# mlaprise/mfrec

Hardware: NVIDIA B200
Metric: rating_updates_per_s (higher is better)
Workload: dtype f32

## Files before the change

### mfrec_b200/csrc/sgd.cu

```cuda
#include <algorithm>
#include <cmath>
#include <cstdlib>
#include <cstring>
#include <thread>
#include <type_traits>

#include <cuda_bf16.h>
#include <cuda_fp16.h>

#include "common.cuh"

namespace {

constexpr int kChunk = 64;
constexpr int kStages = 4;
constexpr int kDepth = 16;
constexpr int kQuadsAhead = kDepth / 4;
constexpr int kRing = kChunk * kStages;
static_assert(kChunk % 4 == 0, "chunks must be 16-byte multiples");
static_assert(4 * kDepth <= kChunk, "the prefetch cursor may run at most one chunk ahead");

struct SgdRank {
    const PackedRating *packed;
    const int64_t *bucket_off;
    const int32_t *col_start;
    float *Q, *ib, *P, *ub;
    double *se_part;
    int32_t *ticks;
    float *peer_Q, *peer_ib;
    int32_t *peer_ticks;
    int32_t *abort;
    int rank;
};

struct SgdParams {
    SgdRank self;
    const SgdRank *ranks;
    int64_t it_begin, it_end;
    int64_t e_base;
    int se_stride;
    int B, W, G, world;
    int tile_rows;
    float lr, Ku, Ki, Kb;
    int update_users, update_items;
    float fx_scale, fx_inv;
    unsigned long long wait_ns;
};

template <int BYTES>
__device__ __forceinline__ void cp_async(void *dst_smem, const void *src_gmem)
{
    if constexpr (BYTES == 16)
        asm volatile("cp.async.cg.shared.global [%0], [%1], 16;" ::"r"(smem_u32(dst_smem)), "l"(src_gmem) : "memory");
    else
        asm volatile("cp.async.ca.shared.global [%0], [%1], %2;" ::"r"(smem_u32(dst_smem)), "l"(src_gmem), "n"(BYTES) : "memory");
}
__device__ __forceinline__ void cp_async_commit() { asm volatile("cp.async.commit_group;" ::: "memory"); }
template <int N>
__device__ __forceinline__ void cp_async_wait() { asm volatile("cp.async.wait_group %0;" ::"n"(N) : "memory"); }

template <int E>
struct Frag {
    static constexpr int V = E >= 4 ? 4 : E;
    static constexpr int NV = E / V;
    float x[E];
};

template <int E>
__device__ __forceinline__ void frag_load(Frag<E> &f, const float *row, int lane)
{
    constexpr int V = Frag<E>::V, NV = Frag<E>::NV;
#pragma unroll
    for (int c = 0; c < NV; ++c) {
        const float *p = row + (c * 32 + lane) * V;
        if constexpr (V == 4) {
            const float4 t = *reinterpret_cast<const float4 *>(p);
            f.x[c * 4 + 0] = t.x; f.x[c * 4 + 1] = t.y; f.x[c * 4 + 2] = t.z; f.x[c * 4 + 3] = t.w;
        } else if constexpr (V == 2) {
            const float2 t = *reinterpret_cast<const float2 *>(p);
            f.x[0] = t.x; f.x[1] = t.y;
        } else {
            f.x[0] = *p;
        }
    }
}

template <int E>
__device__ __forceinline__ void frag_store(const Frag<E> &f, float *row, int lane)
{
    constexpr int V = Frag<E>::V, NV = Frag<E>::NV;
#pragma unroll
    for (int c = 0; c < NV; ++c) {
        float *p = row + (c * 32 + lane) * V;
        if constexpr (V == 4)
            *reinterpret_cast<float4 *>(p) = make_float4(f.x[c * 4], f.x[c * 4 + 1], f.x[c * 4 + 2], f.x[c * 4 + 3]);
        else if constexpr (V == 2)
            *reinterpret_cast<float2 *>(p) = make_float2(f.x[0], f.x[1]);
        else
            *p = f.x[0];
    }
}

template <int E>
__device__ __forceinline__ void frag_store_lane(const Frag<E> &f, float *p)
{
    constexpr int V = Frag<E>::V, NV = Frag<E>::NV;
#pragma unroll
    for (int c = 0; c < NV; ++c) {
        if constexpr (V == 4)
            *reinterpret_cast<float4 *>(p + c * 128) = make_float4(f.x[c * 4], f.x[c * 4 + 1], f.x[c * 4 + 2], f.x[c * 4 + 3]);
        else if constexpr (V == 2)
            *reinterpret_cast<float2 *>(p) = make_float2(f.x[0], f.x[1]);
        else
            *p = f.x[0];
    }
}

template <typename T>
__device__ __forceinline__ T *row_ptr(T *base, uint32_t idx, uint32_t stride_bytes)
{
    uint64_t a;
    asm("mad.wide.u32 %0, %1, %2, %3;" : "=l"(a) : "r"(idx), "r"(stride_bytes), "l"(base));
    return reinterpret_cast<T *>(a);
}

template <int E, typename PT>
__device__ __forceinline__ void pfrag_load(Frag<E> &f, const PT *row, int lane)
{
    if constexpr (sizeof(PT) == 4) {
        frag_load<E>(f, reinterpret_cast<const float *>(row), lane);
    } else {
        constexpr int V = Frag<E>::V, NV = Frag<E>::NV;
        static_assert(V >= 2, "16-bit rows need at least two elements per lane");
#pragma unroll
        for (int c = 0; c < NV; ++c) {
            const PT *p = row + (c * 32 + lane) * V;
#pragma unroll
            for (int h = 0; h < V / 2; ++h) {
                float2 t;
                if constexpr (std::is_same<PT, __half>::value)
                    t = __half22float2(*reinterpret_cast<const __half2 *>(p + 2 * h));
                else
                    t = __bfloat1622float2(*reinterpret_cast<const __nv_bfloat162 *>(p + 2 * h));
                f.x[c * V + 2 * h] = t.x;
                f.x[c * V + 2 * h + 1] = t.y;
            }
        }
    }
}

template <int E, typename PT>
__device__ __forceinline__ void pfrag_store_lane(const Frag<E> &f, PT *p, uint32_t &rng)
{
    if constexpr (sizeof(PT) == 4) {
        frag_store_lane<E>(f, reinterpret_cast<float *>(p));
    } else {
        constexpr int V = Frag<E>::V, NV = Frag<E>::NV;
#pragma unroll
        for (int c = 0; c < NV; ++c) {
            uint32_t w[V / 2];
#pragma unroll
            for (int h = 0; h < V / 2; ++h) {
                const float a = f.x[c * V + 2 * h], b = f.x[c * V + 2 * h + 1];
                if constexpr (std::is_same<PT, __half>::value) {
                    const __half2 t = __floats2half2_rn(a, b);
                    w[h] = *reinterpret_cast<const uint32_t *>(&t);
                } else {
                    rng = rng * 1664525u + 1013904223u;
                    const uint32_t ua = __float_as_uint(a) + (rng & 0xffffu);
                    const uint32_t ub = __float_as_uint(b) + (rng >> 16);
                    w[h] = (ua >> 16) | (ub & 0xffff0000u);
                }
            }
            PT *q = p + c * 32 * V;
            if constexpr (V == 4) *reinterpret_cast<uint2 *>(q) = make_uint2(w[0], w[1]);
            else *reinterpret_cast<uint32_t *>(q) = w[0];
        }
    }
}

__device__ __forceinline__ unsigned long long pack2(float lo, float hi)
{
    unsigned long long r;
    asm("mov.b64 %0, {%1, %2};" : "=l"(r) : "f"(lo), "f"(hi));
    return r;
}
__device__ __forceinline__ void unpack2(unsigned long long v, float &lo, float &hi)
{
    asm("mov.b64 {%0, %1}, %2;" : "=f"(lo), "=f"(hi) : "l"(v));
}
__device__ __forceinline__ unsigned long long mul2(unsigned long long a, unsigned long long b)
{
    unsigned long long r;
    asm("mul.rn.f32x2 %0, %1, %2;" : "=l"(r) : "l"(a), "l"(b));
    return r;
}
__device__ __forceinline__ unsigned long long fma2(unsigned long long a, unsigned long long b, unsigned long long c)
{
    unsigned long long r;
    asm("fma.rn.f32x2 %0, %1, %2, %3;" : "=l"(r) : "l"(a), "l"(b), "l"(c));
    return r;
}

__device__ __forceinline__ int ld_acquire_sys(const int32_t *p)
{
    int v;
    asm volatile("ld.acquire.sys.global.s32 %0, [%1];" : "=r"(v) : "l"(p) : "memory");
    return v;
}
__device__ __forceinline__ void st_release_sys(int32_t *p, int v)
{
    asm volatile("st.release.sys.global.s32 [%0], %1;" ::"l"(p), "r"(v) : "memory");
}
__device__ __forceinline__ unsigned long long global_ns()
{
    unsigned long long t;
    asm volatile("mov.u64 %0, %globaltimer;" : "=l"(t));
    return t;
}

template <int E, int KERNEL, int MAXT, bool GATED, bool RING, typename PT = float>
__global__ void __launch_bounds__(MAXT, 1)
sgd_block_kernel(const SgdParams prm)
{
    constexpr int KPAD = E * 32;
    constexpr unsigned FULL = 0xffffffffu;
    extern __shared__ __align__(128) unsigned char smem_raw[];
    const int W = prm.W;
    const int warp = threadIdx.x >> 5, lane = threadIdx.x & 31;
    const int rb = RING ? (int)(blockIdx.x % (unsigned)prm.B) : (int)blockIdx.x;
    const SgdRank R = RING ? prm.ranks[blockIdx.x / (unsigned)prm.B] : prm.self;
    __shared__ int abort_s;

    float *Qs = reinterpret_cast<float *>(smem_raw);
    float *ibs = Qs + (size_t)prm.tile_rows * KPAD;
    PT *prow_all = reinterpret_cast<PT *>(ibs + ((prm.tile_rows + 3) & ~3));
    float *pbias_all = reinterpret_cast<float *>(prow_all + (size_t)W * kDepth * KPAD);
    PackedRating *ring_all = reinterpret_cast<PackedRating *>(pbias_all + (size_t)W * kDepth);
    uint64_t *bars = reinterpret_cast<uint64_t *>(ring_all + (size_t)W * kRing);
    int64_t *boff = reinterpret_cast<int64_t *>(bars + 1 + kStages * W);
    double *se_s = reinterpret_cast<double *>(boff + W * W + 2);
    volatile int32_t *phase_done = reinterpret_cast<volatile int32_t *>(se_s + W);

    PT *prow = prow_all + (size_t)warp * kDepth * KPAD;
    float *pbias = pbias_all + warp * kDepth;
    PackedRating *ring = ring_all + (size_t)warp * kRing;
    uint64_t *tile_bar = bars;
    uint64_t *my_bar = bars + 1 + kStages * warp;

    if (threadIdx.x == 0) {
        mbar_init(tile_bar, 1);
        for (int i = 0; i < kStages * W; ++i) mbar_init(bars + 1 + i, 1);
        for (int i = 0; i < W; ++i) phase_done[i] = 0;
        abort_s = 0;
        asm volatile("fence.mbarrier_init.release.cluster;" ::: "memory");
    }

    const float lr = prm.lr;
    const bool upd_u = !GATED || prm.update_users != 0, upd_i = !GATED || prm.update_items != 0;
    const float a_i = upd_i ? 1.f - prm.lr * prm.Ki : 1.f;
    const float a_u = upd_u ? 1.f - prm.lr * prm.Ku : 1.f;
    const float a_b = 1.f - prm.lr * prm.Kb;
    const unsigned long long a_i2 = pack2(a_i, a_i), a_u2 = pack2(a_u, a_u);
    const bool upd_bu = (KERNEL == MFREC_KERNEL_LINEAR) || upd_u;
    const bool upd_bi = (KERNEL == MFREC_KERNEL_LINEAR) || upd_i;
    const float fx_scale = prm.fx_scale, fx_inv = prm.fx_inv;
    constexpr uint32_t kRowBytes = KPAD * sizeof(PT);
    PT *const P_rows = reinterpret_cast<PT *>(R.P);
    PT *const P_lane = P_rows + lane * Frag<E>::V;
    uint32_t rng = 0x9e3779b9u * (blockIdx.x * 1024u + threadIdx.x + 1u);
    float *const ub_g = R.ub;
    const int64_t steps_per_epoch = (int64_t)prm.G * prm.B;

    double se = 0.0;
    uint32_t chunk_seq = 0;
    uint32_t tile_seq = 0;
    bool chunks_issued = false;

    int s, t_slab, epoch_rel;
    {
        const int64_t e0 = prm.it_begin / steps_per_epoch;
        const int in0 = (int)(prm.it_begin - e0 * steps_per_epoch);
        epoch_rel = (int)(e0 - prm.e_base);
        t_slab = in0 / prm.B;
        s = in0 - t_slab * prm.B;
    }
    for (int64_t it = prm.it_begin; it < prm.it_end; ++it) {
        const int step = (int)(it - prm.it_begin);
        const int in_epoch = t_slab * prm.B + s;
        int slab = R.rank + t_slab;
        if (slab >= prm.G) slab -= prm.G;
        int cbl = rb + s;
        if (cbl >= prm.B) cbl -= prm.B;
        const int cbg = slab * prm.B + cbl;
        const int cs = R.col_start[cbg * W];
        const int nq = R.col_start[(cbg + 1) * W] - cs;
        const int tick_need = RING ? (int)it : epoch_rel * prm.B + s;

        const int64_t bucket_base = (((int64_t)slab * prm.B + rb) * prm.B + cbl) * W * W;
        for (int i = threadIdx.x; i <= W * W; i += blockDim.x) boff[i] = R.bucket_off[bucket_base + i];
        if (threadIdx.x == 0) {
            if (R.ticks) {
                if constexpr (RING) {
                    const unsigned long long t0 = global_ns();
                    uint32_t polls = 0;
                    while (ld_acquire_sys(R.ticks + cbg) < tick_need) {
                        __nanosleep(128);
                        if ((++polls & 1023u) == 0) {
                            if (*(volatile int32_t *)R.abort) { abort_s = 1; break; }
                            if (prm.wait_ns && global_ns() - t0 > prm.wait_ns) {
                                *(volatile int32_t *)R.abort = 1;
                                abort_s = 1;
                                break;
                            }
                        }
                    }
                } else {
                    while (ld_acquire_gpu(R.ticks + cbg) < tick_need) __nanosleep(64);
                }
                asm volatile("fence.proxy.async;" ::: "memory");
            }
            bool go = nq > 0;
            if constexpr (RING) go = go && !abort_s;
            if (go) {
                const uint32_t total = (uint32_t)nq * KPAD * 4u;
                mbar_expect_tx(tile_bar, total);
                const char *src = reinterpret_cast<const char *>(R.Q + (size_t)cs * KPAD);
                char *dst = reinterpret_cast<char *>(Qs);
                for (uint32_t o = 0; o < total; o += 32768u)
                    bulk_g2s(dst + o, src + o, min(32768u, total - o), tile_bar);
            }
        }
        __syncthreads();
        if constexpr (RING) {
            if (abort_s) break;
        }

        const int64_t S0 = boff[warp * W];
        const uint32_t slen = (uint32_t)(boff[warp * W + W] - S0);
        const uint32_t nchunks = (slen + kChunk - 1) / kChunk;
        const uint32_t nquads = slen / 4;
        const PackedRating *stream = R.packed + S0;
        const int64_t *off_w = boff + warp * W;

        constexpr uint32_t kRingQ = kRing / 4, kChunkQ = kChunk / 4;
        static_assert((kRingQ & (kRingQ - 1)) == 0 && (kChunkQ & (kChunkQ - 1)) == 0 &&
                      (kQuadsAhead & (kQuadsAhead - 1)) == 0, "ring sizes must be powers of two");
        const uint32_t base_q = (chunk_seq % kStages) * kChunkQ;
        const char *const ring_b = reinterpret_cast<const char *>(ring);
        auto quad_rec = [&](uint32_t x) { return ring_b + ((base_q + x) & (kRingQ - 1)) * 48u; };
        auto chunk_wait = [&](uint32_t c) {
            const uint32_t g = chunk_seq + c;
            mbar_wait(my_bar + (g % kStages), (g / kStages) & 1u);
        };
        auto issue_chunk = [&](uint32_t c) {
            if (lane == 0) {
                const uint32_t cnt = min((uint32_t)kChunk, slen - c * kChunk);
                const uint32_t g = chunk_seq + c;
                uint64_t *bar = my_bar + (g % kStages);
                mbar_expect_tx(bar, cnt * 12u);
                bulk_g2s(ring + (g % kStages) * kChunk, stream + (size_t)c * kChunk, cnt * 12u, bar);
            }
        };
        if (!chunks_issued)
            for (uint32_t c = 0; c < nchunks && c < (uint32_t)kStages; ++c) issue_chunk(c);

        PT *const prow_lane = prow + lane * Frag<E>::V;
        for (uint32_t fx = 0; fx + 1 < (uint32_t)kQuadsAhead; ++fx) {
            if (fx < nquads) {
                if ((fx & (kChunkQ - 1)) == 0) chunk_wait(fx / kChunkQ);
                const char *rec = quad_rec(fx);
                const uint32_t fslot0 = (fx & (kQuadsAhead - 1)) * 4;
#pragma unroll
                for (int t = 0; t < 4; ++t) {
                    const uint32_t ut = *reinterpret_cast<const uint32_t *>(rec + 12 * t) & kIdMask;
                    const PT *gsrc = row_ptr(P_lane, ut, kRowBytes);
#pragma unroll
                    for (int c = 0; c < Frag<E>::NV; ++c)
                        cp_async<Frag<E>::V * sizeof(PT)>(prow_lane + (fslot0 + t) * KPAD + c * 32 * Frag<E>::V,
                                                          gsrc + c * 32 * Frag<E>::V);
                }
                if (lane < 4) {
                    const uint32_t ul = *reinterpret_cast<const uint32_t *>(rec + 12 * lane) & kIdMask;
                    cp_async<4>(pbias + fslot0 + lane, row_ptr(ub_g, ul, 4));
                }
            }
            cp_async_commit();
        }

        if (nq > 0) {
            mbar_wait(tile_bar, tile_seq & 1u);
            tile_seq += 1;
        }
        for (int i = threadIdx.x; i < nq; i += blockDim.x) ibs[i] = __ldcg(R.ib + cs + i);
        __syncthreads();

        Frag<E> cp, cq;
#pragma unroll
        for (int e = 0; e < E; ++e) { cp.x[e] = 0.f; cq.x[e] = 0.f; }
        float cbu = 0.f, cbi = 0.f, se_f = 0.f;
        int prev_u = -1, prev_i = -1;

        auto warp_sum_fx = [&](int v) { return __reduce_add_sync(FULL, v); };
        auto dot_fx = [&](const Frag<E> &pu, const Frag<E> &q) {
            float part;
            if constexpr (E >= 2) {
                unsigned long long acc = mul2(pack2(pu.x[0], pu.x[1]), pack2(q.x[0], q.x[1]));
#pragma unroll
                for (int e = 2; e < E; e += 2)
                    acc = fma2(pack2(pu.x[e], pu.x[e + 1]), pack2(q.x[e], q.x[e + 1]), acc);
                float lo, hi;
                unpack2(acc, lo, hi);
                part = lo + hi;
            } else {
                part = pu.x[0] * q.x[0];
            }
            return __float2int_rn(part * fx_scale);
        };
        auto apply = [&](int isum, float r, Frag<E> &pu, float &bu, Frag<E> &q, float &bi) {
            const float pred = fmaf((float)isum, fx_inv, bi + bu);
            float err, grad;
            if constexpr (KERNEL == MFREC_KERNEL_LINEAR) {
                err = r - pred;
                grad = err;
            } else {
                const float sig = 1.f / (1.f + expf(-pred));
                err = r - (1.f + 4.f * sig);
                grad = err * sig * (1.f - sig) * 4.f;
            }
            se_f = fmaf(err, err, se_f);
            const float gl = lr * grad;
            bu = upd_bu ? fmaf(a_b, bu, gl) : bu;
            bi = upd_bi ? fmaf(a_b, bi, gl) : bi;
            const float gli = upd_i ? gl : 0.f, glu = upd_u ? gl : 0.f;
            if constexpr (E >= 2) {
                const unsigned long long glu2 = pack2(glu, glu), gli2 = pack2(gli, gli);
#pragma unroll
                for (int e = 0; e < E; e += 2) {
                    const unsigned long long pe = pack2(pu.x[e], pu.x[e + 1]), qe = pack2(q.x[e], q.x[e + 1]);
                    unpack2(fma2(glu2, qe, mul2(a_u2, pe)), pu.x[e], pu.x[e + 1]);
                    unpack2(fma2(gli2, pe, mul2(a_i2, qe)), q.x[e], q.x[e + 1]);
                }
            } else {
                const float pe = pu.x[0], qe = q.x[0];
                pu.x[0] = fmaf(glu, qe, a_u * pe);
                q.x[0] = fmaf(gli, pe, a_i * qe);
            }
        };
        auto store_p_row = [&](int u, const Frag<E> &pu) {
            pfrag_store_lane<E, PT>(pu, row_ptr(P_lane, (uint32_t)u, kRowBytes), rng);
        };
        auto store_p = [&](int u, const Frag<E> &pu, float bu) {
            store_p_row(u, pu);
            if (lane == 0) *row_ptr(ub_g, (uint32_t)u, 4) = bu;
        };
        auto store_bias_quad = [&](const int (&u4)[4], const float (&b4)[4], uint32_t keep) {
            const bool lo = (lane & 2) == 0, even = (lane & 1) == 0;
            const int ul = lo ? (even ? u4[0] : u4[1]) : (even ? u4[2] : u4[3]);
            const float v = lo ? (even ? b4[0] : b4[1]) : (even ? b4[2] : b4[3]);
            if (lane < 4 && ((keep >> lane) & 1u)) *row_ptr(ub_g, (uint32_t)ul, 4) = v;
        };
        auto store_q = [&](int it, const Frag<E> &q, float bi) {
            frag_store<E>(q, Qs + (size_t)(it - cs) * KPAD, lane);
            if (lane == 0) ibs[it - cs] = bi;
        };

        auto update_one = [&](uint32_t slot, int u, int it, float r, bool stale) {
            Frag<E> pu;
            float bu;
            if (u == prev_u) {
#pragma unroll
                for (int e = 0; e < E; ++e) pu.x[e] = cp.x[e];
                bu = cbu;
            } else if (stale) {
                __syncwarp();
                pfrag_load<E, PT>(pu, row_ptr(P_rows, (uint32_t)u, kRowBytes), lane);
                bu = *row_ptr(ub_g, (uint32_t)u, 4);
            } else {
                pfrag_load<E, PT>(pu, prow + slot * KPAD, lane);
                bu = pbias[slot];
            }
            if (it != prev_i) {
                frag_load<E>(cq, Qs + (size_t)(it - cs) * KPAD, lane);
                cbi = ibs[it - cs];
            }
            const int isum = warp_sum_fx(dot_fx(pu, cq));
            apply(isum, r, pu, bu, cq, cbi);
            store_q(it, cq, cbi);
            store_p(u, pu, bu);
#pragma unroll
            for (int e = 0; e < E; ++e) cp.x[e] = pu.x[e];
            cbu = bu;
            prev_u = u;
            prev_i = it;
        };

        auto load_quad_p = [&](uint32_t slot0, Frag<E> (&p4)[4], float (&b4)[4]) {
#pragma unroll
            for (int t = 0; t < 4; ++t) {
                pfrag_load<E, PT>(p4[t], prow + (slot0 + t) * KPAD, lane);
                b4[t] = pbias[slot0 + t];
            }
        };
        auto chain_quad = [&](uint32_t slot0, const int (&u4)[4], int it, const float (&r4)[4], auto &&hook) {
            Frag<E> p4[4];
            float b4[4];
            load_quad_p(slot0, p4, b4);
            if (it != prev_i) {
                frag_load<E>(cq, Qs + (size_t)(it - cs) * KPAD, lane);
                cbi = ibs[it - cs];
            }
#pragma unroll
            for (int t = 0; t < 4; ++t) {
                const int isum = warp_sum_fx(dot_fx(p4[t], cq));
                hook(t);
                apply(isum, r4[t], p4[t], b4[t], cq, cbi);
                store_p_row(u4[t], p4[t]);
            }
            store_bias_quad(u4, b4, 0xfu);
            store_q(it, cq, cbi);
#pragma unroll
            for (int e = 0; e < E; ++e) cp.x[e] = p4[3].x[e];
            cbu = b4[3];
            prev_u = u4[3];
            prev_i = it;
        };
        auto indep_quad = [&](uint32_t slot0, const int (&u4)[4], const int (&i4)[4], const float (&r4)[4], auto &&hook) {
            Frag<E> p4[4], q4[4];
            float b4[4], c4[4];
            load_quad_p(slot0, p4, b4);
#pragma unroll
            for (int t = 0; t < 4; ++t) {
                frag_load<E>(q4[t], Qs + (size_t)(i4[t] - cs) * KPAD, lane);
                c4[t] = ibs[i4[t] - cs];
            }
            int f[4], sm[4];
#pragma unroll
            for (int t = 0; t < 4; ++t) f[t] = dot_fx(p4[t], q4[t]);
#pragma unroll
            for (int t = 0; t < 4; ++t) sm[t] = warp_sum_fx(f[t]);
#pragma unroll
            for (int t = 0; t < 4; ++t) hook(t);
#pragma unroll
            for (int t = 0; t < 4; ++t) apply(sm[t], r4[t], p4[t], b4[t], q4[t], c4[t]);
#pragma unroll
            for (int t = 0; t < 4; ++t) {
                store_q(i4[t], q4[t], c4[t]);
                store_p_row(u4[t], p4[t]);
            }
            store_bias_quad(u4, b4, 0xfu);
#pragma unroll
            for (int e = 0; e < E; ++e) { cp.x[e] = p4[3].x[e]; cq.x[e] = q4[3].x[e]; }
            cbu = b4[3];
            cbi = c4[3];
            prev_u = u4[3];
            prev_i = i4[3];
        };
        auto clean_quad = [&](uint32_t slot0, const int (&u4)[4], const int (&i4)[4], const int (&f4)[4],
                              const float (&r4)[4], auto &&hook) {
            Frag<E> p4[4];
            float b4[4];
            load_quad_p(slot0, p4, b4);
#pragma unroll
            for (int t = 0; t < 4; ++t) {
                if (f4[t] & kFlagAdjUser) {
#pragma unroll
                    for (int e = 0; e < E; ++e) p4[t].x[e] = t ? p4[t ? t - 1 : 0].x[e] : cp.x[e];
                    b4[t] = t ? b4[t ? t - 1 : 0] : cbu;
                }
                if (i4[t] != prev_i) {
                    frag_load<E>(cq, Qs + (size_t)(i4[t] - cs) * KPAD, lane);
                    cbi = ibs[i4[t] - cs];
                }
                prev_i = i4[t];
                const int isum = warp_sum_fx(dot_fx(p4[t], cq));
                hook(t);
                apply(isum, r4[t], p4[t], b4[t], cq, cbi);
                store_q(i4[t], cq, cbi);
                store_p_row(u4[t], p4[t]);
            }
            {
                uint32_t keep = 0x8u;
#pragma unroll
                for (int t = 0; t < 3; ++t) keep |= (f4[t + 1] & kFlagAdjUser) ? 0u : (1u << t);
                store_bias_quad(u4, b4, keep);
            }
#pragma unroll
            for (int e = 0; e < E; ++e) cp.x[e] = p4[3].x[e];
            cbu = b4[3];
            prev_u = u4[3];
            prev_i = i4[3];
        };

        const int32_t done_base = step * W;
        uint32_t x = 0;
        int4 na = make_int4(0, 0, 0, 0), nb = na, nc = na;
        if (nquads > 0) {
            const int4 *nsrc = reinterpret_cast<const int4 *>(quad_rec(0));
            na = nsrc[0]; nb = nsrc[1]; nc = nsrc[2];
        }
        for (int p = 0; p < W; ++p) {
            const uint32_t xe = (uint32_t)(off_w[p + 1] - S0) >> 2;
            if (p > 0) {
                const volatile int32_t *flag = phase_done + (warp + 1 == W ? 0 : warp + 1);
                if (lane == 0) {
                    while (*flag < done_base + p) __nanosleep(32);
                    __threadfence_block();
                }
                __syncwarp();
            }
            se_f = 0.f;
#pragma unroll 1
            for (; x < xe; ++x) {
                if ((x & (kChunkQ - 1)) == 0 && x != 0) {
                    const uint32_t nc = x / kChunkQ - 1 + kStages;
                    if (nc < nchunks) {
                        __syncwarp();
                        issue_chunk(nc);
                    }
                }
                const uint32_t fx = x + (kQuadsAhead - 1);
                if ((fx & (kChunkQ - 1)) == 0 && fx < nquads) chunk_wait(fx / kChunkQ);
                const char *const frec = quad_rec(min(fx, nquads - 1));
                const uint32_t fu[4] = {*reinterpret_cast<const uint32_t *>(frec) & kIdMask,
                                        *reinterpret_cast<const uint32_t *>(frec + 12) & kIdMask,
                                        *reinterpret_cast<const uint32_t *>(frec + 24) & kIdMask,
                                        *reinterpret_cast<const uint32_t *>(frec + 36) & kIdMask};
                const uint32_t fslot0 = (fx & (kQuadsAhead - 1)) * 4;
                PT *const fdst = prow_lane + fslot0 * KPAD;
                auto fetch_row = [&](int t) {
                    const PT *gsrc = row_ptr(P_lane, fu[t], kRowBytes);
#pragma unroll
                    for (int c = 0; c < Frag<E>::NV; ++c)
                        cp_async<Frag<E>::V * sizeof(PT)>(fdst + t * KPAD + c * 32 * Frag<E>::V, gsrc + c * 32 * Frag<E>::V);
                };
                cp_async_wait<kQuadsAhead - 2>();
                __syncwarp();
                const int4 a = na, b = nb, c2 = nc;
                {
                    const int4 *nsrc = reinterpret_cast<const int4 *>(quad_rec(x + 1));
                    na = nsrc[0]; nb = nsrc[1]; nc = nsrc[2];
                }
                const uint32_t slot0 = (x & (kQuadsAhead - 1)) * 4;
                const int u4[4] = {a.x & kIdMask, a.w & kIdMask, b.z & kIdMask, c2.y & kIdMask};
                const int f4[4] = {a.y, b.x, b.w, c2.z};
                const int i4[4] = {a.y & kIdMask, b.x & kIdMask, b.w & kIdMask, c2.z & kIdMask};
                const float r4[4] = {__int_as_float(a.z), __int_as_float(b.y), __int_as_float(c2.x), __int_as_float(c2.w)};
                const int qtype = (a.x >> kQuadShift) & 3;
                if (qtype == kQuadIndep) {
                    indep_quad(slot0, u4, i4, r4, fetch_row);
                } else if (qtype == kQuadChain) {
                    chain_quad(slot0, u4, i4[0], r4, fetch_row);
                } else if (qtype == kQuadClean) {
                    clean_quad(slot0, u4, i4, f4, r4, fetch_row);
                } else {
#pragma unroll
                    for (int t = 0; t < 4; ++t) {
                        if (!(f4[t] & kFlagPad)) update_one(slot0 + t, u4[t], i4[t], r4[t], (f4[t] & kFlagStale) != 0);
                        fetch_row(t);
                    }
                }
                {
                    const bool lo = (lane & 2) == 0, even = (lane & 1) == 0;
                    const uint32_t ul = lo ? (even ? fu[0] : fu[1]) : (even ? fu[2] : fu[3]);
                    if (lane < 4) cp_async<4>(pbias + fslot0 + lane, row_ptr(ub_g, ul, 4));
                }
                cp_async_commit();
            }
            se += (double)se_f;
            prev_i = -1;
            __syncwarp();
            if (lane == 0) {
                __threadfence_block();
                phase_done[warp] = done_base + p + 1;
            }
        }
        cp_async_wait<0>();
        chunk_seq += nchunks;
        chunks_issued = false;
        int ns = s + 1, nt = t_slab;
        if (ns == prm.B) {
            ns = 0;
            nt = t_slab + 1 == prm.G ? 0 : t_slab + 1;
        }
        if (it + 1 < prm.it_end) {
            int nslab = R.rank + nt;
            if (nslab >= prm.G) nslab -= prm.G;
            int ncbl = rb + ns;
            if (ncbl >= prm.B) ncbl -= prm.B;
            const int64_t nbase = ((((int64_t)nslab * prm.B + rb) * prm.B + ncbl) * W + warp) * W;
            const int64_t nS0 = __ldg(R.bucket_off + nbase);
            const uint32_t nslen = (uint32_t)(__ldg(R.bucket_off + nbase + W) - nS0);
            const uint32_t nn = min((nslen + kChunk - 1) / kChunk, (uint32_t)kStages);
            if (lane == 0) {
                for (uint32_t c = 0; c < nn; ++c) {
                    const uint32_t cnt = min((uint32_t)kChunk, nslen - c * kChunk);
                    const uint32_t g = chunk_seq + c;
                    uint64_t *bar = my_bar + (g % kStages);
                    mbar_expect_tx(bar, cnt * 12u);
                    bulk_g2s(ring + (g % kStages) * kChunk, R.packed + nS0 + (size_t)c * kChunk, cnt * 12u, bar);
                }
            }
            chunks_issued = true;
        }
        __syncthreads();
        const bool to_peer = RING && s + 1 == prm.B && prm.world > 1;
        {
            const int nvec = nq * KPAD / 4;
            float4 *dst = reinterpret_cast<float4 *>((to_peer ? R.peer_Q : R.Q) + (size_t)cs * KPAD);
            float *dst_b = (to_peer ? R.peer_ib : R.ib) + cs;
            const float4 *srcv = reinterpret_cast<const float4 *>(Qs);
            float chk = 0.f;
            for (int i = threadIdx.x; i < nvec; i += blockDim.x) {
                const float4 t = srcv[i];
                chk = fmaf(0.f, t.x, fmaf(0.f, t.y, fmaf(0.f, t.z, fmaf(0.f, t.w, chk))));
                dst[i] = t;
            }
            for (int i = threadIdx.x; i < nq; i += blockDim.x) {
                chk = fmaf(0.f, ibs[i], chk);
                dst_b[i] = ibs[i];
            }
            if (__any_sync(FULL, chk != chk)) se = NAN;
        }
        const bool epoch_ends = in_epoch + 1 == (int)steps_per_epoch || it + 1 == prm.it_end;
        if (epoch_ends) {
            if (lane == 0) se_s[warp] = se;
            se = 0.0;
        }
        if (R.ticks) {
            if constexpr (RING) {
                if (to_peer) {
                    __threadfence_system();
                    __syncthreads();
                    if (threadIdx.x == 0) st_release_sys(R.peer_ticks + cbg, tick_need + 1);
                } else {
                    __threadfence();
                    __syncthreads();
                    if (threadIdx.x == 0) st_release_gpu(R.ticks + cbg, tick_need + 1);
                }
            } else {
                __threadfence();
                __syncthreads();
                if (threadIdx.x == 0) st_release_gpu(R.ticks + cbg, tick_need + 1);
            }
        } else {
            __syncthreads();
        }
        if (epoch_ends && threadIdx.x == 0) {
            double tot = 0.0;
            for (int w = 0; w < W; ++w) tot += se_s[w];
            R.se_part[(int64_t)epoch_rel * prm.se_stride + rb] = tot;
        }
        if (ns == 0 && nt == 0) epoch_rel += 1;
        s = ns;
        t_slab = nt;
    }
    if constexpr (RING) {
        if (abort_s && threadIdx.x == 0) {
            const int64_t e_last = (prm.it_end - 1) / steps_per_epoch;
            for (int64_t e = prm.e_base; e <= e_last; ++e) R.se_part[(e - prm.e_base) * prm.se_stride + rb] = NAN;
        }
    }
}

__global__ void __launch_bounds__(1024) se_reduce_kernel(const double *__restrict__ part, int64_t n,
                                                         double *__restrict__ out)
{
    __shared__ double sh[1024];
    double acc = 0.0;
    for (int64_t i = threadIdx.x; i < n; i += 1024) acc += part[i];
    sh[threadIdx.x] = acc;
    __syncthreads();
    for (int o = 512; o > 0; o >>= 1) {
        if ((int)threadIdx.x < o) sh[threadIdx.x] += sh[threadIdx.x + o];
        __syncthreads();
    }
    if (threadIdx.x == 0) *out = sh[0];
}

__global__ void __launch_bounds__(256)
merge_copies_kernel(float *__restrict__ Q, float *__restrict__ ib, int kpad, const int32_t *__restrict__ hot_off,
                    const int32_t *__restrict__ hot_rows, int32_t n_hot, int32_t row_lo, int32_t row_hi,
                    const int32_t *ticks, int32_t tick_lo, int32_t tick_hi, int32_t tick_need,
                    int32_t *abort_flag, unsigned long long wait_ns)
{
    __shared__ int ok;
    if (ticks) {
        if (threadIdx.x == 0) {
            ok = 1;
            const unsigned long long t0 = global_ns();
            for (int32_t c = tick_lo; c < tick_hi && ok; ++c) {
                uint32_t polls = 0;
                while (ld_acquire_sys(ticks + c) < tick_need) {
                    __nanosleep(256);
                    if ((++polls & 255u) == 0 &&
                        (*(volatile int32_t *)abort_flag || (wait_ns && global_ns() - t0 > wait_ns))) {
                        *(volatile int32_t *)abort_flag = 1;
                        ok = 0;
                        break;
                    }
                }
            }
        }
        __syncthreads();
        if (!ok) return;
    }
    const int lane = threadIdx.x & 31;
    const int64_t warps = ((int64_t)gridDim.x * blockDim.x) >> 5;
    for (int64_t h = ((int64_t)blockIdx.x * blockDim.x + threadIdx.x) >> 5; h < n_hot; h += warps) {
        const int32_t a = hot_off[h], b = hot_off[h + 1];
        const int32_t first = hot_rows[a];
        if (first < row_lo || first >= row_hi) continue;
        const float inv = 1.f / (float)(b - a);
        for (int c = lane; c < kpad; c += 32) {
            float acc = 0.f;
            for (int32_t j = a; j < b; ++j) acc += __ldcg(Q + (size_t)hot_rows[j] * kpad + c);
            acc *= inv;
            for (int32_t j = a; j < b; ++j) Q[(size_t)hot_rows[j] * kpad + c] = acc;
        }
        if (lane == 0) {
            float acc = 0.f;
            for (int32_t j = a; j < b; ++j) acc += __ldcg(ib + hot_rows[j]);
            acc *= inv;
            for (int32_t j = a; j < b; ++j) ib[hot_rows[j]] = acc;
        }
    }
}

constexpr int kSeqRegs = 32;

__global__ void __launch_bounds__(32)
kmf_sequential_kernel(int kernel, int nbr_epochs, int dim, double lr, double K_users,
                      double K_items, double K_bias, double *u, double *v,
                      const int32_t *idx, const double *ratings, int64_t nnz,
                      int64_t ni, int64_t nu, double *ib, double *ub,
                      int update_users, int update_items, double *rmse_out)
{
    if (blockIdx.x != 0) return;
    const int lane = threadIdx.x;
    const unsigned FULLM = 0xffffffffu;
    for (int epoch = 0; epoch < nbr_epochs; ++epoch) {
        double se = 0.0;
        int2 ui = make_int2(0, 0);
        double rating = 0.0;
        if (lane < nnz) { ui = reinterpret_cast<const int2 *>(idx)[lane]; rating = ratings[lane]; }
        for (int64_t base = 0; base < nnz; base += 32) {
            const int cnt = (int)(nnz - base < 32 ? nnz - base : 32);
            const bool live = lane < cnt;
            const int user = ui.x, item = ui.y;
            const double r = rating;
            {
                const int64_t j = base + 32 + lane;
                if (j < nnz) { ui = reinterpret_cast<const int2 *>(idx)[j]; rating = ratings[j]; }
            }
            int lmax;
            const int level = mfrec_window_levels(user, item, live, lane, lmax);
            double e2 = 0.0;
            for (int L = 1; L <= lmax; ++L) {
                if (live && level == L) {
                    double *const ui_ = u + item, *const vu_ = v + user;
                    const double bi0 = ib[item], bu0 = ub[user];
                    double s = __dadd_rn(__dadd_rn(0.0, bi0), bu0);
                    auto err_grad = [&](double &err, double &grad) {
                        if (kernel == MFREC_KERNEL_LINEAR) {
                            err = __dadd_rn(r, -s);
                            grad = err;
                        } else {
                            const double sig = 1.0 / __dadd_rn(1.0, exp(-s));
                            const double p = __dadd_rn(1.0, __dmul_rn(sig, 4.0));
                            err = __dadd_rn(r, -p);
                            grad = __dmul_rn(__dmul_rn(__dmul_rn(err, sig), __dadd_rn(1.0, -sig)), 4.0);
                        }
                        e2 = __dmul_rn(err, err);
                        if (kernel == MFREC_KERNEL_LINEAR || update_users)
                            ub[user] = __dadd_rn(bu0, __dmul_rn(lr, __dadd_rn(grad, -__dmul_rn(K_bias, bu0))));
                        if (kernel == MFREC_KERNEL_LINEAR || update_items)
                            ib[item] = __dadd_rn(bi0, __dmul_rn(lr, __dadd_rn(grad, -__dmul_rn(K_bias, bi0))));
                    };
                    double err, grad;
                    if (dim <= kSeqRegs) {
                        double mf[kSeqRegs], cf[kSeqRegs];
#pragma unroll
                        for (int f = 0; f < kSeqRegs; ++f)
                            if (f < dim) { mf[f] = ui_[(int64_t)f * ni]; cf[f] = vu_[(int64_t)f * nu]; }
#pragma unroll
                        for (int f = 0; f < kSeqRegs; ++f)
                            if (f < dim) s = __dadd_rn(s, __dmul_rn(mf[f], cf[f]));
                        err_grad(err, grad);
#pragma unroll
                        for (int f = 0; f < kSeqRegs; ++f) {
                            if (f >= dim) continue;
                            if (update_items)
                                ui_[(int64_t)f * ni] =
                                    __dadd_rn(mf[f], __dmul_rn(lr, __dadd_rn(__dmul_rn(grad, cf[f]), -__dmul_rn(K_items, mf[f]))));
                            if (update_users)
                                vu_[(int64_t)f * nu] =
                                    __dadd_rn(cf[f], __dmul_rn(lr, __dadd_rn(__dmul_rn(grad, mf[f]), -__dmul_rn(K_users, cf[f]))));
                        }
                    } else {
                        for (int f0 = 0; f0 < dim; f0 += 8) {
                            double a[8], b[8];
#pragma unroll
                            for (int j = 0; j < 8; ++j)
                                if (f0 + j < dim) { a[j] = ui_[(int64_t)(f0 + j) * ni]; b[j] = vu_[(int64_t)(f0 + j) * nu]; }
#pragma unroll
                            for (int j = 0; j < 8; ++j)
                                if (f0 + j < dim) s = __dadd_rn(s, __dmul_rn(a[j], b[j]));
                        }
                        err_grad(err, grad);
                        for (int f0 = 0; f0 < dim; f0 += 8) {
                            double mf[8], cf[8];
#pragma unroll
                            for (int j = 0; j < 8; ++j)
                                if (f0 + j < dim) { mf[j] = ui_[(int64_t)(f0 + j) * ni]; cf[j] = vu_[(int64_t)(f0 + j) * nu]; }
#pragma unroll
                            for (int j = 0; j < 8; ++j) {
                                if (f0 + j >= dim) continue;
                                if (update_items)
                                    ui_[(int64_t)(f0 + j) * ni] =
                                        __dadd_rn(mf[j], __dmul_rn(lr, __dadd_rn(__dmul_rn(grad, cf[j]), -__dmul_rn(K_items, mf[j]))));
                                if (update_users)
                                    vu_[(int64_t)(f0 + j) * nu] =
                                        __dadd_rn(cf[j], __dmul_rn(lr, __dadd_rn(__dmul_rn(grad, mf[j]), -__dmul_rn(K_users, cf[j]))));
                            }
                        }
                    }
                }
                __syncwarp();
            }
            for (int t = 0; t < cnt; ++t) se = __dadd_rn(se, __shfl_sync(FULLM, e2, t));
        }
        if (rmse_out && lane == 0) rmse_out[epoch] = sqrt(se / (double)nnz);
        __syncwarp();
    }
}

}

size_t mfrec_sgd_smem_bytes(int tile_rows, int kpad, int W, int p_elem_bytes)
{
    size_t b = (size_t)tile_rows * kpad * 4;
    b += (size_t)((tile_rows + 3) & ~3) * 4;
    b += (size_t)W * kDepth * kpad * p_elem_bytes;
    b += (size_t)W * kDepth * 4;
    b += (size_t)W * kRing * sizeof(PackedRating);
    b += (size_t)(1 + kStages * W) * 8;
    b += (size_t)(W * W + 2) * 8;
    b += (size_t)W * 8;
    b += (size_t)((W + 3) & ~3) * 4;
    return b + 384;
}

namespace {

template <int E>
int launch_sgd(mfrec_ctx *ctx, int kernel, SgdParams &prm, size_t smem, bool cooperative, int grid, bool ring,
               int p_kind)
{
    const bool wide = prm.W > 8;
    const bool gated = !(prm.update_users && prm.update_items);
    void (*fn)(const SgdParams) = nullptr;
    const bool mid = prm.W > 8 && prm.W <= 12 && !gated;
#define MF_PICK(K)                                                                                     \
    fn = mid ? sgd_block_kernel<E, K, 384, false, false>                                                \
       : wide ? (gated ? sgd_block_kernel<E, K, 512, true, false> : sgd_block_kernel<E, K, 512, false, false>) \
              : (gated ? sgd_block_kernel<E, K, 256, true, false> : sgd_block_kernel<E, K, 256, false, false>)
#define MF_PICK_RING(K) \
    fn = mid ? sgd_block_kernel<E, K, 384, false, true>                                                  \
       : wide ? sgd_block_kernel<E, K, 512, false, true> : sgd_block_kernel<E, K, 256, false, true>
    if (p_kind != MFREC_STORAGE_F32) {
        if constexpr (E >= 2) {
            if (ring || gated || prm.W > 12)
                return mfrec_set_error(ctx, MFREC_ERR_UNSUPPORTED,
                                       "fp16 / bf16 user-factor storage: single device, both sides updated, at most 12 warps per CTA");
#define MF_PICK16(K, T) fn = prm.W > 8 ? sgd_block_kernel<E, K, 384, false, false, T> : sgd_block_kernel<E, K, 256, false, false, T>
            if (kernel == MFREC_KERNEL_LINEAR) {
                if (p_kind == MFREC_STORAGE_F16) { MF_PICK16(MFREC_KERNEL_LINEAR, __half); } else { MF_PICK16(MFREC_KERNEL_LINEAR, __nv_bfloat16); }
            } else {
                if (p_kind == MFREC_STORAGE_F16) { MF_PICK16(MFREC_KERNEL_LOGISTIC, __half); } else { MF_PICK16(MFREC_KERNEL_LOGISTIC, __nv_bfloat16); }
            }
#undef MF_PICK16
        } else {
            return mfrec_set_error(ctx, MFREC_ERR_UNSUPPORTED, "fp16 / bf16 user-factor storage needs k > 32");
        }
    } else if (ring) {
        if (gated)
            return mfrec_set_error(ctx, MFREC_ERR_UNSUPPORTED, "ring launches train both sides");
        if (kernel == MFREC_KERNEL_LINEAR) { MF_PICK_RING(MFREC_KERNEL_LINEAR); } else { MF_PICK_RING(MFREC_KERNEL_LOGISTIC); }
    } else {
        if (kernel == MFREC_KERNEL_LINEAR) { MF_PICK(MFREC_KERNEL_LINEAR); } else { MF_PICK(MFREC_KERNEL_LOGISTIC); }
    }
#undef MF_PICK
#undef MF_PICK_RING
    MF_CUDA(ctx, cudaFuncSetAttribute(fn, cudaFuncAttributeMaxDynamicSharedMemorySize, (int)smem));
    if (cooperative) {
        void *args[] = {(void *)&prm};
        MF_CUDA(ctx, cudaLaunchCooperativeKernel((const void *)fn, dim3(grid), dim3(prm.W * 32), args, smem,
                                                 ctx->stream));
        ctx->launches += 1;
    } else {
        fn<<<grid, prm.W * 32, smem, ctx->stream>>>(prm);
        MF_LAUNCH_CHECK(ctx);
    }
    return MFREC_OK;
}

int launch_sgd_kpad(mfrec_ctx *ctx, int kpad, int kernel, SgdParams &prm, size_t smem, bool cooperative,
                    int grid = 0, bool ring = false, int p_kind = MFREC_STORAGE_F32)
{
    if (grid == 0) grid = prm.B;
    switch (kpad) {
    case 32: return launch_sgd<1>(ctx, kernel, prm, smem, cooperative, grid, ring, p_kind);
    case 64: return launch_sgd<2>(ctx, kernel, prm, smem, cooperative, grid, ring, p_kind);
    case 128: return launch_sgd<4>(ctx, kernel, prm, smem, cooperative, grid, ring, p_kind);
    case 256: return launch_sgd<8>(ctx, kernel, prm, smem, cooperative, grid, ring, p_kind);
    default: return mfrec_set_error(ctx, MFREC_ERR_UNSUPPORTED, "kpad=%d", kpad);
    }
}

bool sgd_fits_one_wave(mfrec_ctx *ctx, int n, int W, size_t smem)
{
    if (n <= ctx->sm_count) return smem <= ctx->smem_optin;
    const size_t per_sm = ctx->smem_per_sm;
    const int by_smem = (int)(per_sm / (smem + 1024));
    const int by_threads = 2048 / (W * 32);
// ... 607 lines not shown
```

Baseline: 6.358 billion.

## Write back item-factor slices per warp with bulk async copies, dropping block barrier

Each warp now writes back only the item-factor group it last touched (the previous warp's column group), using a TMA bulk shared-to-global copy for the local case instead of a block-wide float4 loop. The write-back happens right after the warp's own phase completes, and the __syncthreads before the copy is removed, so warps can overlap the write-back with prefetching the next step's chunks. This relies on the phase-done ordering guaranteeing group glast is finished by the time warp reaches this point, and the NaN check now runs per warp over its slice. Peer writes still use the scalar loop.

```diff
diff --git a/mfrec_b200/csrc/sgd.cu b/mfrec_b200/csrc/sgd.cu
--- a/mfrec_b200/csrc/sgd.cu
+++ b/mfrec_b200/csrc/sgd.cu
@@ -58,6 +58,13 @@
 __device__ __forceinline__ void cp_async_commit() { asm volatile("cp.async.commit_group;" ::: "memory"); }
 template <int N>
 __device__ __forceinline__ void cp_async_wait() { asm volatile("cp.async.wait_group %0;" ::"n"(N) : "memory"); }
+__device__ __forceinline__ void bulk_s2g(void *dst_gmem, const void *src_smem, uint32_t bytes)
+{
+    asm volatile("cp.async.bulk.global.shared::cta.bulk_group [%0], [%1], %2;" ::"l"(dst_gmem), "r"(smem_u32(src_smem)),
+                 "r"(bytes)
+                 : "memory");
+}
+
 
 template <int E>
 struct Frag {
@@ -295,6 +302,8 @@
         const int cbg = slab * prm.B + cbl;
         const int cs = R.col_start[cbg * W];
         const int nq = R.col_start[(cbg + 1) * W] - cs;
+        const int glast = warp == 0 ? W - 1 : warp - 1;
+        const int g0 = R.col_start[cbg * W + glast] - cs, g1 = R.col_start[cbg * W + glast + 1] - cs;
         const int tick_need = RING ? (int)it : epoch_rel * prm.B + s;
 
         const int64_t bucket_base = (((int64_t)slab * prm.B + rb) * prm.B + cbl) * W * W;
@@ -677,6 +686,34 @@
         }
         cp_async_wait<0>();
         chunk_seq += nchunks;
+        const bool to_peer = RING && s + 1 == prm.B && prm.world > 1;
+        {
+            const uint32_t bytes = (uint32_t)(g1 - g0) * KPAD * 4u;
+            float *const dst = (to_peer ? R.peer_Q : R.Q) + (size_t)(cs + g0) * KPAD;
+            float *const dst_b = (to_peer ? R.peer_ib : R.ib) + cs;
+            const float *const src = Qs + (size_t)g0 * KPAD;
+            if (!to_peer && bytes > 0) {
+                asm volatile("fence.proxy.async.shared::cta;" ::: "memory");
+                __syncwarp();
+                if (lane == 0) {
+                    for (uint32_t o = 0; o < bytes; o += 32768u)
+                        bulk_s2g(reinterpret_cast<char *>(dst) + o, reinterpret_cast<const char *>(src) + o,
+                                 min(32768u, bytes - o));
+                    asm volatile("cp.async.bulk.commit_group;" ::: "memory");
+                }
+            }
+            float chk = 0.f;
+            for (uint32_t i = lane; i < bytes / 16u; i += 32) {
+                const float4 t = reinterpret_cast<const float4 *>(src)[i];
+                chk = fmaf(0.f, t.x, fmaf(0.f, t.y, fmaf(0.f, t.z, fmaf(0.f, t.w, chk))));
+                if (to_peer) reinterpret_cast<float4 *>(dst)[i] = t;
+            }
+            for (int i = g0 + lane; i < g1; i += 32) {
+                chk = fmaf(0.f, ibs[i], chk);
+                dst_b[i] = ibs[i];
+            }
+            if (__any_sync(FULL, chk != chk)) se = NAN;
+        }
         chunks_issued = false;
         int ns = s + 1, nt = t_slab;
         if (ns == prm.B) {
@@ -703,24 +740,9 @@
             }
             chunks_issued = true;
         }
-        __syncthreads();
-        const bool to_peer = RING && s + 1 == prm.B && prm.world > 1;
-        {
-            const int nvec = nq * KPAD / 4;
-            float4 *dst = reinterpret_cast<float4 *>((to_peer ? R.peer_Q : R.Q) + (size_t)cs * KPAD);
-            float *dst_b = (to_peer ? R.peer_ib : R.ib) + cs;
-            const float4 *srcv = reinterpret_cast<const float4 *>(Qs);
-            float chk = 0.f;
-            for (int i = threadIdx.x; i < nvec; i += blockDim.x) {
-                const float4 t = srcv[i];
-                chk = fmaf(0.f, t.x, fmaf(0.f, t.y, fmaf(0.f, t.z, fmaf(0.f, t.w, chk))));
-                dst[i] = t;
-            }
-            for (int i = threadIdx.x; i < nq; i += blockDim.x) {
-                chk = fmaf(0.f, ibs[i], chk);
-                dst_b[i] = ibs[i];
-            }
-            if (__any_sync(FULL, chk != chk)) se = NAN;
+        if (lane == 0) {
+            asm volatile("cp.async.bulk.wait_group 0;" ::: "memory");
+            asm volatile("fence.proxy.async.global;" ::: "memory");
         }
         const bool epoch_ends = in_epoch + 1 == (int)steps_per_epoch || it + 1 == prm.it_end;
         if (epoch_ends) {
```

New measurement: 6.367 billion (median of 6 runs). Within noise of the previous version (+0.1%).
